# cvxopt/smcp

Hardware: AMD Instinct MI355X
Metric: Newton KKT solves/sec (higher is better)
Workload: dtype f64; 1 GPU; synth50k nested block-arrow SDP n=50000, 8073 cliques, m=100; kktsolver=chol, n=50000, cliques=8073, m=100, blkval_doubles=2493568, update_doubles=10689536, parallelism=single

## Files before the change

smcp_amd/csrc/constraints.cpp:

```cpp
#include "constraints.hpp"

#include <algorithm>
#include <atomic>

#include "../../include/smcp_amd.h"
#include "hostpar.hpp"

namespace smcp {
namespace {

struct Build {
  const Symbolic& S;
  const ConstraintParams& P;
  const int64_t m, nnz;
  const int64_t* cptr;
  const int64_t* cidx;
  const double* cval;
  ConstraintTables& T;
  std::vector<int32_t> ek, eoff;
  int threads = 1;
};

bool locate_entries(Build& B) {
  const Symbolic& S = B.S;
  ConstraintTables& T = B.T;
  const int64_t nnz = B.nnz;
  const int64_t* cidx = B.cidx;
  const double* cval = B.cval;
  T.w.resize(nnz); T.ar.resize(nnz); T.ac.resize(nnz);
  B.ek.resize(nnz); B.eoff.resize(nnz);
  const int nth = B.threads = host_threads(B.P.max_threads, nnz / 65536 + 1);
  std::atomic<int> bad{0};
  auto work = [&](int tix) {
    const int64_t e0 = nnz * tix / nth, e1 = nnz * (tix + 1) / nth;
    int64_t k = 0;
    for (int64_t e = e0; e < e1; ++e) {
      int64_t pos = cidx[e];
      if (pos < 0 || pos >= S.blklen()) { bad = 1; return; }
      if (pos < S.blkptr[k] || pos >= S.blkptr[k + 1])
        k = (int64_t)(std::upper_bound(S.blkptr.begin(), S.blkptr.end(), pos) - S.blkptr.begin()) - 1;
      int64_t nf = S.nf(k), off = pos - S.blkptr[k];
      int64_t col = off / nf, row = off % nf;
      if (row < col) { bad = 1; return; }
      T.w[e] = (row == col) ? cval[e] : 2.0 * cval[e];
      T.ar[e] = (int32_t)S.rowidx[S.rowptr[k] + row];
      T.ac[e] = (int32_t)(S.snptr[k] + col);
      B.ek[e] = (int32_t)k;
      B.eoff[e] = (int32_t)off;
    }
  };
  run_threads(nth, work);
  return !bad;
}

void classify_columns(Build& B) {
  const Symbolic& S = B.S;
  const ConstraintParams& P = B.P;
  ConstraintTables& T = B.T;
  const int64_t m = B.m, nnz = B.nnz;
  const int64_t* cptr = B.cptr;
  T.rloc.assign(nnz, 0); T.cloc.assign(nnz, 0);
  T.h_kptr.assign(1, 0);
  const int64_t tnz = (int64_t)((double)S.n * P.tnzcols);
  const int64_t colcap = ((int64_t)256 << 20) / std::max<int64_t>(1, S.n * 8);
  const int64_t kcap = std::min<int64_t>(tnz, std::max<int64_t>(1, colcap));
  const int64_t sepsum = std::max<int64_t>(1, S.sepptr[S.nsn]);
  const int64_t trsm_cap = std::max<int64_t>(1, (P.max_rhs * P.tmplen) / sepsum);
  std::vector<std::vector<int32_t>> kss((size_t)m);
  std::vector<char> is_sparse((size_t)m, 0);
  const int64_t cap = std::min(kcap, trsm_cap);
  const int nth = B.threads = host_threads(P.max_threads, m, nnz / 4096 + 1);
  auto work = [&](int tix) {
    for (int64_t j = tix; j < m; j += nth) {
      std::vector<int32_t>& ks = kss[(size_t)j];
      ks.reserve((size_t)(2 * (cptr[j + 1] - cptr[j])));
      for (int64_t e = cptr[j]; e < cptr[j + 1]; ++e) { ks.push_back(T.ar[e]); ks.push_back(T.ac[e]); }
      std::sort(ks.begin(), ks.end());
      ks.erase(std::unique(ks.begin(), ks.end()), ks.end());
      const int64_t nz = (int64_t)ks.size();
      const bool sparse = P.scm_on && nz > 0 && nz <= cap;
      is_sparse[(size_t)j] = sparse ? 1 : 0;
      if (!sparse) { std::vector<int32_t>().swap(ks); continue; }
      for (int64_t e = cptr[j]; e < cptr[j + 1]; ++e) {
        T.rloc[e] = (int32_t)(std::lower_bound(ks.begin(), ks.end(), T.ar[e]) - ks.begin());
        T.cloc[e] = (int32_t)(std::lower_bound(ks.begin(), ks.end(), T.ac[e]) - ks.begin());
      }
    }
  };
  run_threads(nth, work);
  int64_t kmax = 1;
  for (int64_t j = 0; j < m; ++j) {
    if (!is_sparse[(size_t)j]) { T.dl.push_back((int32_t)j); continue; }
    T.sl.push_back((int32_t)j);
    T.kidx.insert(T.kidx.end(), kss[(size_t)j].begin(), kss[(size_t)j].end());
    T.h_kptr.push_back((int64_t)T.kidx.size());
    kmax = std::max(kmax, (int64_t)kss[(size_t)j].size());
  }
  if (!T.sl.empty()) T.vcols = std::min(trsm_cap, std::max(kmax, std::min<int64_t>((int64_t)T.kidx.size(), colcap)));
}

void csr_by_position(Build& B) {
  ConstraintTables& T = B.T;
  const int64_t m = B.m, nnz = B.nnz;
  const int64_t* cptr = B.cptr;
  const int64_t* cidx = B.cidx;
  const double* cval = B.cval;
  T.rcon.resize(nnz); T.rval.resize(nnz);
  std::vector<int32_t> con(nnz);
  for (int64_t j = 0; j < m; ++j)
    for (int64_t e = cptr[j]; e < cptr[j + 1]; ++e) con[e] = (int32_t)j;
  const int nth = B.threads = host_threads(B.P.max_threads, nnz / 65536 + 1);
  const int64_t P = B.S.blklen();
  std::vector<std::vector<int64_t>> start((size_t)nth);
  std::vector<int64_t> ecount((size_t)nth + 1, 0), dcount((size_t)nth + 1, 0);
  auto count = [&](int tix) {
    const int64_t p0 = P * tix / nth, p1 = P * (tix + 1) / nth;
    std::vector<int64_t>& st = start[(size_t)tix];
    st.assign((size_t)(p1 - p0) + 1, 0);
    for (int64_t e = 0; e < nnz; ++e) { const int64_t p = cidx[e]; if (p >= p0 && p < p1) ++st[(size_t)(p - p0) + 1]; }
    int64_t distinct = 0;
    for (int64_t p = 0; p < p1 - p0; ++p) { distinct += st[(size_t)p + 1] != 0; st[(size_t)p + 1] += st[(size_t)p]; }
    ecount[(size_t)tix + 1] = st[(size_t)(p1 - p0)];
    dcount[(size_t)tix + 1] = distinct;
  };
  run_threads(nth, count);
  for (int t = 0; t < nth; ++t) { ecount[(size_t)t + 1] += ecount[(size_t)t]; dcount[(size_t)t + 1] += dcount[(size_t)t]; }
  T.rpos.resize((size_t)dcount[(size_t)nth]);
  T.rptr.resize((size_t)dcount[(size_t)nth] + 1);
  auto place = [&](int tix) {
    const int64_t p0 = P * tix / nth, p1 = P * (tix + 1) / nth, q0 = ecount[(size_t)tix];
    std::vector<int64_t>& st = start[(size_t)tix];
    int64_t d = dcount[(size_t)tix];
    for (int64_t p = 0; p < p1 - p0; ++p)
      if (st[(size_t)p + 1] != st[(size_t)p]) { T.rpos[(size_t)d] = p0 + p; T.rptr[(size_t)d] = q0 + st[(size_t)p]; ++d; }
    for (int64_t e = 0; e < nnz; ++e) {
      const int64_t p = cidx[e];
      if (p < p0 || p >= p1) continue;
      const int64_t q = q0 + st[(size_t)(p - p0)]++;
      T.rcon[(size_t)q] = con[e];
      T.rval[(size_t)q] = cval[e];
    }
  };
  run_threads(nth, place);
  T.rptr[(size_t)dcount[(size_t)nth]] = nnz;
}

void group_entries(Build& B) {
  const Symbolic& S = B.S;
  ConstraintTables& T = B.T;
  const int64_t m = B.m, nnz = B.nnz;
  const int64_t* cptr = B.cptr;
  const std::vector<int32_t>& ek = B.ek;
  const std::vector<int32_t>& eoff = B.eoff;
  std::vector<int32_t>& kptr = T.kptr;
  kptr.assign((size_t)(S.nsn * (m + 1)) + 1, 0);
  T.koff.resize(nnz); T.kval.resize(nnz); T.kij.resize(nnz);
  const int nth = B.threads = host_threads(B.P.max_threads, m, nnz / 65536 + 1);
  auto over_constraints = [&](auto body) {
    run_threads(nth, [&](int tix) { for (int64_t j = tix; j < m; j += nth) body(j); });
  };
  over_constraints([&](int64_t j) {
    for (int64_t e = cptr[j]; e < cptr[j + 1]; ++e) kptr[(size_t)ek[e] * (m + 1) + j + 1]++;
  });
  int64_t run = 0;
  for (int64_t k = 0; k < S.nsn; ++k) {
    for (int64_t j = 0; j <= m; ++j) {
      const size_t idx = (size_t)k * (m + 1) + j;
      const int32_t cnt = (j < m) ? kptr[idx + 1] : 0;
      kptr[idx] = (int32_t)run;
      if (j < m) run += cnt;
    }
  }
  std::vector<int32_t> fill(kptr.begin(), kptr.end() - 1);
  over_constraints([&](int64_t j) {
    for (int64_t e = cptr[j]; e < cptr[j + 1]; ++e) {
      const int64_t nf = S.nf(ek[e]);
      const int32_t q = fill[(size_t)ek[e] * (m + 1) + j]++;
      T.koff[q] = eoff[e];
      T.kval[q] = B.cval[e];
      T.kij[q] = (int32_t)((eoff[e] % nf) & 0xffff) | (int32_t)((eoff[e] / nf) << 16);
    }
  });
  kptr.pop_back();
  T.kc_sorted = true;
  for (size_t q = 0; q + 1 < kptr.size() && T.kc_sorted; ++q)
    for (int32_t e = kptr[q] + 1; e < kptr[q + 1]; ++e)
      if (T.koff[(size_t)e] <= T.koff[(size_t)e - 1]) { T.kc_sorted = false; break; }
}

void entry_statistics(Build& B) {
  const Symbolic& S = B.S;
  ConstraintTables& T = B.T;
  const int64_t m = B.m;
  const std::vector<int64_t>& fam = *B.P.fam;
  auto len = [&](int64_t k, int64_t j) { const size_t q = (size_t)k * (m + 1) + j; return (int64_t)(T.kptr[q + 1] - T.kptr[q]); };
  T.kc_maxlist = 0;
  for (int64_t k = 0; k < S.nsn; ++k)
    if (S.nn(k) <= 16 && S.na(k) <= 64)
      for (int64_t j = 0; j < m; ++j) T.kc_maxlist = std::max(T.kc_maxlist, len(k, j));
  int64_t sum = 0, pairs = 0;
  for (int64_t k = 0; k < S.nsn; ++k)
    if (k < (int64_t)fam.size() && fam[k] == 2)
      for (int64_t j = 0; j < m; ++j) {
        int64_t tot = len(k, j);
        for (int64_t q2 = S.chptr[k]; q2 < S.chptr[k + 1]; ++q2) tot += len(S.chidx[q2], j);
        T.fam_maxterms = std::max(T.fam_maxterms, tot);
        sum += tot;
        ++pairs;
      }
  if (pairs) T.fam_meanterms = (double)sum / (double)pairs;
  T.kc_maxlist_large = 0;
  for (int64_t k = 0; k < S.nsn; ++k)
    if ((S.nn(k) > 16 || S.na(k) > 64) && S.nn(k) <= 64 && S.na(k) <= 128 && S.chptr[k + 1] == S.chptr[k])
      for (int64_t j = 0; j < m; ++j) T.kc_maxlist_large = std::max(T.kc_maxlist_large, len(k, j));
  T.lg_slot_of.assign((size_t)S.nsn, -1);
  T.lg_eptr.assign(1, 0);
  for (int64_t k = 0; k < S.nsn; ++k)
    if (k < (int64_t)fam.size() && fam[k] == 1) {
      const int64_t E = T.kptr[(size_t)k * (m + 1) + m] - T.kptr[(size_t)k * (m + 1)];
      T.lg_slot_of[(size_t)k] = (int32_t)T.lg_children++;
      T.lg_maxent = std::max(T.lg_maxent, E);
      T.lg_pairs += E * (E + 1) / 2;
      T.lg_rows += S.nf(k) * S.nn(k);
      T.lg_rec = std::max<int>(T.lg_rec, (int)(S.nf(k) * S.nf(k) + S.nf(k) * S.nn(k)));
      T.lg_eptr.push_back(T.lg_eptr.back() + (int32_t)E);
    }
}

void leafgram_lists(Build& B) {
  ConstraintTables& T = B.T;
  const int64_t m = B.m;
  T.epk.resize((size_t)T.lg_eptr.back());
  T.ewv.resize((size_t)T.lg_eptr.back());
  T.remap.assign((size_t)m, -1);
  for (int64_t k = 0; k < B.S.nsn; ++k) {
    const int32_t g = T.lg_slot_of[(size_t)k];
    if (g < 0) continue;
    int32_t o = T.lg_eptr[(size_t)g];
    for (int64_t j = 0; j < m; ++j)
      for (int32_t q = T.kptr[(size_t)k * (m + 1) + j]; q < T.kptr[(size_t)k * (m + 1) + j + 1]; ++q, ++o) {
        const int32_t i = T.kij[q] & 0xffff, jc = T.kij[q] >> 16;
        T.epk[(size_t)o] = i | (jc << 8) | ((int32_t)j << 16);
        T.ewv[(size_t)o] = i == jc ? 0.5 * T.kval[q] : T.kval[q];
      }
  }
  for (size_t q = 0; q < T.dl.size(); ++q) T.remap[(size_t)T.dl[q]] = (int32_t)q;
  T.has_leafgram = true;
}

bool number_families(Build& B) {
  const Symbolic& S = B.S;
  const ConstraintParams& P = B.P;
  ConstraintTables& T = B.T;
  T.fno.assign((size_t)S.nsn, -1);
  T.fz_levels.assign((size_t)S.nlev, 0);
  T.has_fz_levels = true;
  int64_t nfam = 0;
  bool ok = true;
  for (int64_t k = 0; k < S.nsn; ++k)
    if ((*P.fam)[(size_t)k] == 2) {
      T.fno[(size_t)k] = (int32_t)nfam++;
      const int64_t par = S.snpar[k];
      if (par < 0 || (size_t)par >= P.large_mask->size() || !(*P.large_mask)[(size_t)par] || S.nf(par) > P.lf_alds_maxnf) ok = false;
      else T.fz_levels[(size_t)S.level[(size_t)par]] = 1;
    }
  T.fz_nfam = nfam;
  return ok && nfam > 0 && nfam < ((int64_t)1 << 19) && nfam * (B.m + 1) < ((int64_t)1 << 31);
}

void family_term_lists(Build& B) {
  const Symbolic& S = B.S;
  ConstraintTables& T = B.T;
  const int64_t m = B.m, nfam = T.fz_nfam;
  const int32_t CHILD = B.P.famt_child;
  const std::vector<int32_t>& kptr = T.kptr;
  const std::vector<int32_t>& kij = T.kij;
  const std::vector<double>& kval = T.kval;
  std::vector<int32_t>& fptr = T.fptr;
  fptr.assign((size_t)(nfam * (m + 1)) + 1, 0);
  std::vector<int64_t> fam_k((size_t)nfam);
  int64_t run = 0;
  for (int64_t k = 0; k < S.nsn; ++k) {
    const int32_t f = T.fno[(size_t)k];
    if (f < 0) continue;
    fam_k[(size_t)f] = k;
    for (int64_t j = 0; j < m; ++j) {
      fptr[(size_t)f * (m + 1) + j] = (int32_t)run;
      run += kptr[(size_t)k * (m + 1) + j + 1] - kptr[(size_t)k * (m + 1) + j];
      for (int64_t q2 = S.chptr[k]; q2 < S.chptr[k + 1]; ++q2) {
        const size_t q = (size_t)S.chidx[q2] * (m + 1) + j;
        run += kptr[q + 1] - kptr[q];
      }
    }
    fptr[(size_t)f * (m + 1) + m] = (int32_t)run;
  }
  fptr[(size_t)(nfam * (m + 1))] = (int32_t)run;
  T.fpk.resize((size_t)run);
  T.fsv.resize((size_t)run);
  const int nth = B.threads = host_threads(B.P.max_threads, nfam / 16 + 1);
  run_threads(nth, [&](int tix) {
    for (int64_t f = tix; f < nfam; f += nth) {
      const int64_t k = fam_k[(size_t)f];
      for (int64_t j = 0; j < m; ++j) {
        size_t o = (size_t)fptr[(size_t)f * (m + 1) + j];
        for (int32_t q = kptr[(size_t)k * (m + 1) + j]; q < kptr[(size_t)k * (m + 1) + j + 1]; ++q, ++o) {
          const int32_t i = kij[q] & 0xffff, jc = kij[q] >> 16;
          T.fpk[o] = i | (jc << 16);
          T.fsv[o] = i == jc ? 0.5 * kval[q] : kval[q];
        }
        int32_t colbase = 0;
        for (int64_t q2 = S.chptr[k]; q2 < S.chptr[k + 1]; ++q2) {
          const int64_t cc = S.chidx[q2];
          const int32_t nnc = (int32_t)S.nn(cc);
          const int32_t* rel = &S.relidx[S.sepptr[cc]];
          for (int32_t q = kptr[(size_t)cc * (m + 1) + j]; q < kptr[(size_t)cc * (m + 1) + j + 1]; ++q, ++o) {
            const int32_t i = kij[q] & 0xffff, jc = kij[q] >> 16;
            if (i >= nnc) { T.fpk[o] = (CHILD + colbase + jc) | (rel[i - nnc] << 16); T.fsv[o] = -kval[q]; }
            else { T.fpk[o] = (CHILD + colbase + i) | ((CHILD + colbase + jc) << 16); T.fsv[o] = i == jc ? 0.5 * kval[q] : kval[q]; }
          }
          colbase += nnc;
        }
      }
    }
  });
  T.has_fam_terms = true;
}

}

int build_constraint_tables(const Symbolic& S, const ConstraintParams& P, int64_t m, const int64_t* cptr, const int64_t* cidx,
                            const double* cval, ConstraintTables& T, const ConstraintStepMark& mark) {
  T = ConstraintTables();
  Build B{S, P, m, cptr[m], cptr, cidx, cval, T, {}, {}};
  auto done = [&](const char* step) { if (mark) mark(step, B.threads); B.threads = 1; };
  if (!locate_entries(B)) return SMCP_EINVAL;
  done("locate entries");
  classify_columns(B);
  done("classify");
  csr_by_position(B);
  done("CSR by position");
  if (B.nnz < ((int64_t)1 << 31) && S.nsn * (m + 1) <= ((int64_t)1 << 28)) {
    group_entries(B);
    entry_statistics(B);
    T.has_entry_tables = true;
    done("entry tables");
    if (T.lg_children > 0 && m < 32768) leafgram_lists(B);
    done("leaf Gram tables");
    if (T.fam_maxterms > 0 && P.famt_terms_ok(T.fam_maxterms, T.fam_meanterms) && !P.fam->empty() && number_families(B))
      family_term_lists(B);
    done("family term lists");
  }
  return 0;
}

}
```

smcp_amd/csrc/front_famt.hip:

```cpp
#include <hip/hip_runtime.h>

namespace smcp {

struct FamtL { int oLi, onK, onMK, oRt, oZero, oCN, oCA, oCM, total; };
template <int NAT>
__host__ __device__ inline FamtL famt_layout(int ncol) {
  constexpr int NA = 16 * NAT;
  FamtL L{};
  int o = 0;
  L.oLi = o; o += 256;
  L.onK = o; o += NA * 16;
  L.onMK = o; o += NA * 16;
  L.oRt = o; o += NA * NA;
  L.oZero = o; o += NA;
  L.oCN = o; o += ncol * 16;
  L.oCA = o; o += ncol * NA;
  L.oCM = o; o += ncol * NA;
  L.total = o;
  return L;
}
typedef unsigned int famt_u2 __attribute__((ext_vector_type(2)));
__device__ inline __amdgpu_buffer_rsrc_t famt_rsrc(double* base, int doubles) {
  return __builtin_amdgcn_make_buffer_rsrc(base, 0, doubles * 8, 0x00020000);
}
#ifndef SMCP_FAMT_AUX
#define SMCP_FAMT_AUX 0
#endif
__device__ inline void famt_store(__amdgpu_buffer_rsrc_t r, bool ok, int pos, double v) {
  __builtin_amdgcn_raw_buffer_store_b64(__builtin_bit_cast(famt_u2, v), r, ok ? pos * 8 : -1, 0, SMCP_FAMT_AUX);
}
#ifndef SMCP_FAMT_NW
#define SMCP_FAMT_NW 12
#endif
constexpr int FAMT_NW = SMCP_FAMT_NW;
constexpr int FAMT_HDR = 32;
constexpr int FAMT_TCAP = 96;
constexpr int FAMT_TMAX = 384;
constexpr int FAMT_CHILD = 128;

template <int NAT>
__host__ __device__ inline int famt_prep_doubles(int cnn) { constexpr int NA = 16 * NAT; return NA * NA + NA * 16 + 256 + 8 * (NA + 16 + cnn * NA); }

template <int NAT>
__global__ void __launch_bounds__(512) k_famt_prep(MfmaArgs a, double* famt, int cnn, int32_t* fz_slot) {
  extern __shared__ __attribute__((aligned(16))) double smem[];
  constexpr int NA = 16 * NAT;
  const int ncol = 8 * cnn;
  const FamtL L = famt_layout<NAT>(ncol);
  const int k = a.t.lev[blockIdx.x];
  const CliqueDesc d = a.t.cl[k];
  const int nn = d.nn, na = d.na, nf = nn + na, nch = d.chend - d.chbeg;
  const int tid = threadIdx.x, lane = tid & 63, wave = tid >> 6;
  double* const sRt = smem;
  double* const snK = sRt + NA * NA;
  double* const sLi = snK + NA * 16;
  double* const qt = sLi + 256 + wave * (NA + 16 + cnn * NA);
  double* const sCA = qt + NA + 16;
  double* const out = famt + (int64_t)blockIdx.x * (FAMT_HDR + L.total);
  double* const T = out + FAMT_HDR;
  const int myck = lane < nch ? a.t.chidx[d.chbeg + lane] : 0;
  const int mynn = lane < nch ? a.t.cl[myck].nn : 0;
  int inc = mynn;
#pragma unroll
  for (int o = 1; o < 8; o <<= 1) { const int v = __shfl_up(inc, o); if (lane >= o) inc += v; }
  const int colbase = __shfl(inc - mynn, min(wave, 7));
  const int ck = __shfl(myck, min(wave, 7));
  for (int e = tid; e < NA * NA + NA * 16 + 256; e += 512) smem[e] = 0.0;
  __syncthreads();
  {
    const double* lk = a.LK + d.blk;
    const double* ys = a.ysc + d.upd;
    for (int e = tid; e < nf * nn; e += 512) {
      const int i = e % nf, j = e / nf;
      if (i >= nn) snK[(i - nn) + j * NA] = -lk[e];
      else if (i >= j) sLi[i + j * 16] = lk[e];
    }
    batched_loop<8>(tid, na * na, 512, [=](int e) { return ys[e]; },
                    [=](int e, double v) {
                      const int i = e % na, p = e / na;
                      if (i >= p) sRt[p + i * NA] = v;
                    });
  }
  __syncthreads();
  for (int e = tid; e < 256; e += 512) T[L.oLi + e] = sLi[e];
  for (int e = tid; e < NA * 16; e += 512) T[L.onK + e] = snK[e];
  for (int e = tid; e < NA * NA; e += 512) T[L.oRt + e] = sRt[e];
  for (int e = tid; e < NA; e += 512) T[L.oZero + e] = 0.0;
  for (int e = tid; e < NA * 16; e += 512) {
    const int p = e % NA, c = e / NA;
    double s = 0.0;
    if (p < na && c < nn)
      for (int q = p; q < na; ++q) s += sRt[p + q * NA] * snK[q + c * NA];
    T[L.onMK + e] = s;
  }
  if (wave < nch) {
    const CliqueDesc cd = a.t.cl[ck];
    const int nnc = cd.nn, nac = cd.na, nfc = nnc + nac;
    const double* lkc = a.LK + cd.blk;
    const int rel = lane < nac ? a.t.relidx[cd.rel + lane] : 0;
    for (int j = 0; j < nnc; ++j) {
      const double kv = lane < nac ? lkc[(nnc + lane) + (int64_t)j * nfc] : 0.0;
      for (int e = lane; e < NA + 16; e += 64) qt[e] = 0.0;
      __builtin_amdgcn_fence(__ATOMIC_RELEASE, "wavefront"); __builtin_amdgcn_wave_barrier(); __builtin_amdgcn_fence(__ATOMIC_ACQUIRE, "wavefront");
      if (lane < nac) qt[rel < nn ? rel : 16 + (rel - nn)] = kv;
      __builtin_amdgcn_fence(__ATOMIC_RELEASE, "wavefront"); __builtin_amdgcn_wave_barrier(); __builtin_amdgcn_fence(__ATOMIC_ACQUIRE, "wavefront");
      const int g = colbase + j;
      if (lane < 16) {
        double s = 0.0;
        if (lane < nn)
          for (int q = 0; q <= lane; ++q) s += sLi[lane + q * 16] * qt[q];
        T[L.oCN + g * 16 + lane] = s;
      }
      for (int p = lane; p < NA; p += 64) {
        double s = 0.0;
        if (p < na) {
          s = qt[16 + p];
          for (int q = 0; q < nn; ++q) s += snK[p + q * NA] * qt[q];
        }
        sCA[j * NA + p] = s;
        T[L.oCA + g * NA + p] = s;
      }
    }
    __builtin_amdgcn_fence(__ATOMIC_RELEASE, "wavefront"); __builtin_amdgcn_wave_barrier(); __builtin_amdgcn_fence(__ATOMIC_ACQUIRE, "wavefront");
    for (int j0 = 0; j0 < nnc; j0 += 8)
      for (int p = lane; p < NA; p += 64) {
        double s8[8] = {0.0, 0.0, 0.0, 0.0, 0.0, 0.0, 0.0, 0.0};
        if (p < na)
          for (int q = p; q < na; ++q) {
            const double rt = sRt[p + q * NA];
#pragma unroll
            for (int x = 0; x < 8; ++x) s8[x] += rt * sCA[min(j0 + x, cnn - 1) * NA + q];
          }
#pragma unroll
        for (int x = 0; x < 8; ++x) if (j0 + x < nnc) T[L.oCM + (colbase + j0 + x) * NA + p] = s8[x];
      }
    if (lane == 0) {
      int* const hdr = reinterpret_cast<int*>(out) + 16 + 6 * wave;
      hdr[0] = ck; hdr[1] = nnc; hdr[2] = nac; hdr[3] = colbase; hdr[4] = 0; hdr[5] = 0;
    }
  } else if (wave < 8 && lane == 0) {
    int* const hdr = reinterpret_cast<int*>(out) + 16 + 6 * wave;
    hdr[0] = -1; hdr[1] = 1; hdr[2] = 0; hdr[3] = 0; hdr[4] = 0; hdr[5] = 0;
  }
  {
    const int used = __shfl(inc, 7);
    for (int e = tid; e < (ncol - used) * 16; e += 512) T[L.oCN + used * 16 + e] = 0.0;
    for (int e = tid; e < (ncol - used) * NA; e += 512) { T[L.oCA + used * NA + e] = 0.0; T[L.oCM + used * NA + e] = 0.0; }
  }
  if (tid == 0) {
    if (fz_slot && a.fz_no && a.fz_no[k] >= 0) fz_slot[a.fz_no[k]] = (int32_t)blockIdx.x;
    int* const hdr = reinterpret_cast<int*>(out);
    hdr[0] = k; hdr[1] = nn; hdr[2] = na; hdr[3] = nch;
    hdr[4] = (int)(d.blk & 0xffffffffll); hdr[5] = (int)(d.blk >> 32);
    hdr[6] = 0; hdr[7] = 0;
    hdr[8] = (int)(d.updp & 0xffffffffll); hdr[9] = (int)(d.updp >> 32);
  }
}

template <int NTH>
__device__ inline void famt_copy_tables(double* smem, const double* src, int total, int tid) {
  const double2* const s2 = reinterpret_cast<const double2*>(src);
  double2* const d2 = reinterpret_cast<double2*>(smem);
  const int n2 = total >> 1;
  for (int e0 = tid; e0 < n2; e0 += NTH * 8) {
    double2 v[8];
#pragma unroll
    for (int x = 0; x < 8; ++x) v[x] = s2[min(e0 + x * NTH, n2 - 1)];
#pragma unroll
    for (int x = 0; x < 8; ++x) if (e0 + x * NTH < n2) d2[e0 + x * NTH] = v[x];
  }
}

__host__ __device__ inline int famt_desc_doubles() { return FAMT_TCAP * 3; }

template <int NAT, bool UPD = true>
__global__ void __launch_bounds__(64 * FAMT_NW) k_fam_terms(MfmaArgs a, double* u, int64_t ldu, const double* famt, int cnn,
                                                   const int32_t* kc_ij, int tabpasses, int ecap) {
  extern __shared__ __attribute__((aligned(16))) double smem[];
  constexpr int NA = 16 * NAT, NW = FAMT_NW, NTH = 64 * NW;
  const int ncol = 8 * cnn;
  const FamtL L = famt_layout<NAT>(ncol);
  const double* const fc = famt + (int64_t)blockIdx.x * (FAMT_HDR + L.total);
  const int32_t* const hdr = reinterpret_cast<const int32_t*>(fc);
  const int k = hdr[0], nn = hdr[1], na = hdr[2], nch = hdr[3], nf = nn + na;
  const int64_t pblk = (int64_t)(uint32_t)hdr[4] | ((int64_t)hdr[5] << 32);
  const int64_t pupdp = (int64_t)(uint32_t)hdr[8] | ((int64_t)hdr[9] << 32);
  const int tid = threadIdx.x;
  const int lane = tid & 63, l15 = lane & 15, kq = lane >> 4;
  const int wave = __builtin_amdgcn_readfirstlane(tid >> 6);
  const int nmem = nch + 1;
  const int gy = (int)gridDim.y;
  const int npass = ((int)a.nrhs - (int)blockIdx.y + gy - 1) / gy;
  double* const dS = smem + L.total + wave * famt_desc_doubles();
  int* const dI = reinterpret_cast<int*>(dS + FAMT_TCAP);
  int* const misc = reinterpret_cast<int*>(smem + L.total + NW * famt_desc_doubles());
  int* const epfit = misc;
  int* const cdim = misc + 2;
  int* const tab = misc + 12;
  double* const lval = reinterpret_cast<double*>(tab + 2 * ((tabpasses * nmem + 1) & ~1));
  int* const lpk = reinterpret_cast<int*>(lval + ecap);

  famt_copy_tables<NTH>(smem, fc + FAMT_HDR, L.total, tid);
  if (tid < 8) cdim[tid] = tid < nch ? (hdr[16 + 6 * tid + 1] | (hdr[16 + 6 * tid + 3] << 8)) : 1;

  for (int q0 = 0; q0 < npass;) {
    const int epmax = min(tabpasses, npass - q0), npairs = epmax * nmem;
    __syncthreads();
    if (tid == 0) *epfit = epmax;
    int myp0[2] = {0, 0};
#pragma unroll
    for (int h = 0; h < 2; ++h) {
      const int idx = tid + NTH * h;
      if (idx < npairs) {
        const int qq = idx / nmem, mem = idx - qq * nmem;
        const int r = (int)blockIdx.y + (q0 + qq) * gy;
        const int j = a.kc_ids ? a.kc_ids[a.kc_j0 + r] : a.kc_j0 + r;
        const int ck = mem ? hdr[16 + 6 * (mem - 1)] : k;
        const int32_t* kp = a.kc_ptr + (int64_t)ck * a.kc_stride;
        myp0[h] = kp[j];
        tab[2 * idx] = kp[j + 1] - myp0[h];
      }
    }
    __syncthreads();
    if (wave == 0) {
      const int per = (npairs + 63) / 64, b = lane * per;
      int sum = 0;
      for (int x = 0; x < per; ++x) sum += (b + x < npairs) ? tab[2 * (b + x)] : 0;
      int incl = sum;
#pragma unroll
      for (int o = 1; o < 64; o <<= 1) { const int v = __shfl_up(incl, o); if (lane >= o) incl += v; }
      int run = incl - sum;
      for (int x = 0; x < per; ++x)
        if (b + x < npairs) {
          const int c = tab[2 * (b + x)];
          tab[2 * (b + x) + 1] = run;
          run += c;
          if (run > ecap) atomicMin(epfit, (b + x) / nmem);
        }
    }
    __syncthreads();
    const int ep = max(1, *epfit);
#pragma unroll
    for (int h = 0; h < 2; ++h) {
      const int idx = tid + NTH * h;
      if (idx < ep * nmem) {
        const int c = tab[2 * idx], p0 = myp0[h], off = tab[2 * idx + 1];
        const int qq = idx / nmem, mem = idx - qq * nmem;
        (void)qq;
        const int mnn = mem ? hdr[16 + 6 * (mem - 1) + 1] : 0;
        const int mck = mem ? hdr[16 + 6 * (mem - 1)] : 0;
        const int32_t* const mrel = a.t.relidx + a.t.cl[mem ? mck : k].rel;
        for (int t = 0; t < c && off + t < ecap; ++t) {
          const int ij = kc_ij[p0 + t];
          const int i = ij & 0xffff, jc = ij >> 16;
          int pk = i | (jc << 8);
          if (mem && i >= mnn) pk |= mrel[i - mnn] << 16;
          lpk[off + t] = pk;
          lval[off + t] = a.kc_val[p0 + t];
        }
      }
    }
    __builtin_amdgcn_s_waitcnt(0x0F70);
    __syncthreads();

    for (int qq = wave; qq < ep; qq += NW) {
      const int r = (int)blockIdx.y + (q0 + qq) * gy;
      const int* const trow = tab + 2 * qq * nmem;
      int cntm = lane < nmem ? trow[2 * lane] : 0;
      int incl = cntm;
#pragma unroll
      for (int o = 1; o < 16; o <<= 1) { const int v = __shfl_up(incl, o); if (lane >= o) incl += v; }
      const int Ttot = min(__builtin_amdgcn_readlane(incl, 15), FAMT_TMAX);
      const int ndp = max(1, (Ttot + FAMT_TCAP / 2 - 1) / (FAMT_TCAP / 2));
      auto build = [&](int dp) {
        const int e = dp * (FAMT_TCAP / 2) + lane;
        const int T = min(FAMT_TCAP / 2, Ttot - dp * (FAMT_TCAP / 2));
        int mem = 0, base = 0;
#pragma unroll
        for (int mm = 0; mm < 8; ++mm) {
          const int up = __builtin_amdgcn_readlane(incl, mm);
          if (e >= up) { mem = mm + 1; base = up; }
        }
        if (lane < T) {
          const int where = trow[2 * mem + 1];
          const int pk = lpk[where + (e - base)];
          const double v = lval[where + (e - base)];
          const int i = pk & 0xff, jc = (pk >> 8) & 0xff, rl = (pk >> 16) & 0xff;
          int vx, vy;
          double s;
          if (mem == 0) { vx = i; vy = jc; s = i == jc ? 0.5 * v : v; }
          else {
            const int cd = cdim[mem - 1], nnc = cd & 0xff, cb = cd >> 8;
            if (i >= nnc) { vx = FAMT_CHILD + cb + jc; vy = rl; s = -v; }
            else { vx = FAMT_CHILD + cb + i; vy = FAMT_CHILD + cb + jc; s = i == jc ? 0.5 * v : v; }
          }
          auto img = [&](int vid, int& on, int& oa, int& om, int& ui) {
            if (vid >= FAMT_CHILD) { const int g = vid - FAMT_CHILD; on = L.oCN + 16 * g; oa = L.oCA + NA * g; om = L.oCM + NA * g; ui = 255; }
            else if (vid < nn) { on = L.oLi + 16 * vid; oa = L.onK + NA * vid; om = L.onMK + NA * vid; ui = 255; }
            else { on = L.oZero; oa = L.oZero; om = L.oRt + NA * (vid - nn); ui = vid - nn; }
          };
          int nx, ax, mx, ux, ny, ay, my, uy;
          img(vx, nx, ax, mx, ux);
          img(vy, ny, ay, my, uy);
          dS[2 * lane] = s; dS[2 * lane + 1] = s;
          int4 w0 = {nx | (ax << 16), mx | (ux << 16), ny | (ay << 16), uy};
          int4 w1 = {ny | (ay << 16), my | (uy << 16), nx | (ax << 16), ux};
          reinterpret_cast<int4*>(dI)[2 * lane] = w0;
          reinterpret_cast<int4*>(dI)[2 * lane + 1] = w1;
        }
        if (lane < 4 && 2 * T + lane < ((2 * T + 3) & ~3)) {
          dS[2 * T + lane] = 0.0;
          int4 z = {L.oZero | (L.oZero << 16), L.oZero | (255 << 16), L.oZero | (L.oZero << 16), 255};
          reinterpret_cast<int4*>(dI)[2 * T + lane] = z;
        }
        __builtin_amdgcn_fence(__ATOMIC_RELEASE, "wavefront"); __builtin_amdgcn_wave_barrier(); __builtin_amdgcn_fence(__ATOMIC_ACQUIRE, "wavefront");
      };
      build(0);
      const __amdgpu_buffer_rsrc_t rP = famt_rsrc(u + (int64_t)r * ldu + pblk, nf * nn);
      const __amdgpu_buffer_rsrc_t rU = famt_rsrc(a.t.updp + (int64_t)r * a.t.updplen + pupdp, (na * (na + 1)) >> 1);
      bool fresh = true;
      auto pass = [&](auto LOc, auto HIc, auto Gc) {
        constexpr int LO = decltype(LOc)::value, HI = decltype(HIc)::value;
        constexpr bool WITHG = decltype(Gc)::value;
        constexpr int NTU = UPD ? HI * (HI + 1) / 2 - LO * (LO + 1) / 2 : 1;
        d4 accU[NTU], accQ[HI - LO], accG = {0.0, 0.0, 0.0, 0.0};
#pragma unroll
        for (int x = 0; x < NTU; ++x) accU[x] = d4{0.0, 0.0, 0.0, 0.0};
#pragma unroll
        for (int x = 0; x < HI - LO; ++x) accQ[x] = d4{0.0, 0.0, 0.0, 0.0};
        for (int dp = 0; dp < ndp; ++dp) {
        if (!(fresh && dp == 0)) {
          __builtin_amdgcn_fence(__ATOMIC_RELEASE, "wavefront"); __builtin_amdgcn_wave_barrier(); __builtin_amdgcn_fence(__ATOMIC_ACQUIRE, "wavefront");
          build(dp);
        }
        fresh = ndp == 1;
        const int ks = (2 * min(FAMT_TCAP / 2, Ttot - dp * (FAMT_TCAP / 2)) + 3) >> 2;
        for (int s = 0; s < ks; ++s) {
          const int tp = kq + 4 * s;
          const double sc = dS[tp];
          const int4 w = reinterpret_cast<const int4*>(dI)[tp];
          const int nx = w.x & 0xffff, ax = w.x >> 16, mx = w.y & 0xffff, ux = w.y >> 16;
          const int ny = w.z & 0xffff, ay = w.z >> 16, uy = w.w;
          double bA[HI - LO], bM[HI - LO], aA[HI];
#pragma unroll
          for (int t = 0; t < HI; ++t) {
            const int row = 16 * t + l15;
            if constexpr (UPD) aA[t] = sc * (smem[ay + row] + (row == uy ? 1.0 : 0.0));
            if (t >= LO) {
              if constexpr (UPD) bA[t - LO] = smem[ax + row] + (row == ux ? 1.0 : 0.0);
              bM[t - LO] = smem[mx + row];
            }
          }
          const double aN = sc * smem[ny + l15];
#pragma unroll
          for (int rt = LO; rt < HI; ++rt) {
            if constexpr (UPD) {
#pragma unroll
              for (int ct = 0; ct <= rt; ++ct) {
                constexpr int base = LO * (LO + 1) / 2;
                const int x = rt * (rt + 1) / 2 + ct - base;
                accU[x] = __builtin_amdgcn_mfma_f64_16x16x4f64(aA[ct], bA[rt - LO], accU[x], 0, 0, 0);
              }
            }
            accQ[rt - LO] = __builtin_amdgcn_mfma_f64_16x16x4f64(aN, bM[rt - LO], accQ[rt - LO], 0, 0, 0);
          }
          if constexpr (WITHG) {
            const double bN = smem[nx + l15];
            accG = __builtin_amdgcn_mfma_f64_16x16x4f64(aN, bN, accG, 0, 0, 0);
          }
        }
        }
#pragma unroll
        for (int rt = LO; rt < HI; ++rt) {
          const int m = 16 * rt + l15;
          const bool mok = m < na;
          if constexpr (UPD) {
#pragma unroll
            for (int ct = 0; ct <= rt; ++ct)
#pragma unroll
              for (int x = 0; x < 4; ++x) {
                const int n = 16 * ct + kq + 4 * x;
                const int cb = (n * (2 * na - 1 - n)) >> 1;
                famt_store(rU, ct < rt ? mok : (mok && m >= n), cb + m, accU[rt * (rt + 1) / 2 + ct - LO * (LO + 1) / 2][x]);
              }
          }
#pragma unroll
          for (int x = 0; x < 4; ++x) {
            const int n = kq + 4 * x;
            famt_store(rP, mok && n < nn, (nn + m) + n * nf, accQ[rt - LO][x]);
          }
        }
        if constexpr (WITHG) {
#pragma unroll
          for (int x = 0; x < 4; ++x) {
            const int jn = kq + 4 * x;
            famt_store(rP, l15 < nn && jn <= l15, l15 + jn * nf, accG[x]);
          }
        }
      };
      if constexpr (!UPD) {
        pass(std::integral_constant<int, 0>{}, std::integral_constant<int, NAT>{}, std::true_type{});
      } else if constexpr (NAT == 4 && FAMT_NW > 8) {
        pass(std::integral_constant<int, 0>{}, std::integral_constant<int, 2>{}, std::true_type{});
        pass(std::integral_constant<int, 2>{}, std::integral_constant<int, 3>{}, std::false_type{});
        pass(std::integral_constant<int, 3>{}, std::integral_constant<int, 4>{}, std::false_type{});
      } else if constexpr (NAT == 3 && FAMT_NW > 8) {
        pass(std::integral_constant<int, 0>{}, std::integral_constant<int, 2>{}, std::true_type{});
        pass(std::integral_constant<int, 2>{}, std::integral_constant<int, 3>{}, std::false_type{});
      } else if constexpr (NAT == 4) {
        pass(std::integral_constant<int, 0>{}, std::integral_constant<int, 3>{}, std::false_type{});
        pass(std::integral_constant<int, 3>{}, std::integral_constant<int, 4>{}, std::true_type{});
      } else {
        pass(std::integral_constant<int, 0>{}, std::integral_constant<int, NAT>{}, std::true_type{});
      }
    }
    q0 += ep;
  }
}

template <int NAT, int PFG = 1>
__device__ inline void lf_add_family(double* T, int nf, const MfmaArgs& a, int z, int64_t pt, const int32_t* rel, int lane) {
  constexpr int NA = 16 * NAT, NTU = NAT * (NAT + 1) / 2;
  const int l15 = lane & 15, kq = lane >> 4;
  const int slot = z & 0x7ffff, nnp = (z >> 19) & 31, nap = (z >> 24) & 127;
  const FamtL L = famt_layout<NAT>(8 * a.fz_cnn);
  const double* const tab = a.fz_tab + (int64_t)slot * a.fz_recl + FAMT_HDR;
  const int pbase = (int)(uint32_t)(pt & 0xffffffffll), Ttot = min((int)(pt >> 32), FAMT_TMAX);
  int relv[NAT];
#pragma unroll
  for (int t = 0; t < NAT; ++t) relv[t] = rel[min(16 * t + l15, max(nap - 1, 0))];
  d4 acc[NTU];
#pragma unroll
  for (int x = 0; x < NTU; ++x) acc[x] = d4{0.0, 0.0, 0.0, 0.0};
  auto chunk = [&](const int p0, const int Tn) {
  int pk = 0;
  double sv = 0.0;
  if (lane < Tn) { pk = a.fz_pk[p0 + lane]; sv = a.fz_s[p0 + lane]; }
  const int ks = (2 * Tn + 3) >> 2;
  auto fetch = [&](int s, double (&aA)[NAT], double& se, int& ux, int& uy) {
    const int tp = kq + 4 * s, e = tp >> 1;
    const int pke = __shfl(pk, e, 64);
    se = __shfl(sv, e, 64);
    const int v0 = pke & 0xffff, v1 = (pke >> 16) & 0xffff;
    const int vx = (tp & 1) ? v1 : v0, vy = (tp & 1) ? v0 : v1;
    ux = (vx < FAMT_CHILD && vx >= nnp) ? vx - nnp : 255;
    const int ay = vy >= FAMT_CHILD ? L.oCA + NA * (vy - FAMT_CHILD) : (vy < nnp ? L.onK + NA * vy : L.oZero);
    uy = (vy < FAMT_CHILD && vy >= nnp) ? vy - nnp : 255;
#pragma unroll
    for (int t = 0; t < NAT; ++t) aA[t] = tab[ay + 16 * t + l15];
  };
  auto mma = [&](double (&aA)[NAT], double se, int ux, int uy) {
    double bA[NAT];
#pragma unroll
    for (int t = 0; t < NAT; ++t) bA[t] = __shfl_xor(aA[t], 16, 64);
#pragma unroll
    for (int t = 0; t < NAT; ++t) {
      const int row = 16 * t + l15;
      aA[t] = se * (aA[t] + (row == uy ? 1.0 : 0.0));
      bA[t] = bA[t] + (row == ux ? 1.0 : 0.0);
    }
#pragma unroll
    for (int rt = 0; rt < NAT; ++rt)
#pragma unroll
      for (int ct = 0; ct <= rt; ++ct)
        acc[rt * (rt + 1) / 2 + ct] = __builtin_amdgcn_mfma_f64_16x16x4f64(aA[ct], bA[rt], acc[rt * (rt + 1) / 2 + ct], 0, 0, 0);
  };
  if constexpr (PFG == 1) {
    for (int s = 0; s < ks; ++s) {
      double aA[NAT], se;
      int ux, uy;
      fetch(s, aA, se, ux, uy);
      mma(aA, se, ux, uy);
    }
  } else {
    for (int s0 = 0; s0 < ks; s0 += PFG) {
      double aA[PFG][NAT], se[PFG];
      int ux[PFG], uy[PFG];
#pragma unroll
      for (int g = 0; g < PFG; ++g) {
        fetch(min(s0 + g, ks - 1), aA[g], se[g], ux[g], uy[g]);
        if (s0 + g >= ks) se[g] = 0.0;
      }
#pragma unroll
      for (int g = 0; g < PFG; ++g) mma(aA[g], se[g], ux[g], uy[g]);
    }
  }
  };
  if (Ttot <= 64) chunk(pbase, Ttot);
  else for (int c0 = 0; c0 < Ttot; c0 += 64) chunk(pbase + c0, min(64, Ttot - c0));
#pragma unroll
  for (int rt = 0; rt < NAT; ++rt) {
    const int m = 16 * rt + l15;
#pragma unroll
    for (int ct = 0; ct <= rt; ++ct)
#pragma unroll
      for (int x = 0; x < 4; ++x) {
        const int n = 16 * ct + kq + 4 * x;
        const int cj = __shfl(relv[ct], kq + 4 * x, 64);
        const bool ok = m < nap && n < nap && (ct < rt || m >= n);
        if (ok) unsafeAtomicAdd(&T[cj * nf - ((cj * (cj - 1)) >> 1) - cj + relv[rt]], acc[rt * (rt + 1) / 2 + ct][x]);
      }
  }
}
template <int NAT, int PFG = 1>
struct AldsFam {
  const MfmaArgs* a;
  const int64_t* sCu; const int64_t* sCr;
  __device__ void operator()(double* T, int nf, int r, const int* sFz, int nmine, int wave, int nw, int lane) const {
    (void)r;
    for (int qi = wave; qi < nmine; qi += nw) {
      const int z = sFz[qi];
      if (z >= 0) lf_add_family<NAT, PFG>(T, nf, *a, z, sCu[qi], a->t.relidx + sCr[qi], lane);
    }
  }
};
template <int NAT, int NTH>
__global__ void __launch_bounds__(NTH) k_lf_assemble_fz(MfmaArgs a, double* u, int64_t ldu, int sgn, int cnt, int nrhs, int* counters,
                                                        int tail_first, int nzt) {
  extern __shared__ __attribute__((aligned(16))) double T[];
  __shared__ int stask;
  const int64_t* const sCu = reinterpret_cast<const int64_t*>(T + lf_alds_doubles(a.nnmax + a.namax));
  const int64_t* const sCr = sCu + a.nchmax;
  const int q0 = (int)(blockIdx.x & 7);
  for (int dq = 0; dq < 8; ++dq) {
    const int q = (q0 + dq) & 7;
    const int nfq = (cnt - q + 7) >> 3;
    const int total = nfq * nrhs;
    if (total <= 0) continue;
    const int full = (tail_first >= 0 && tail_first < total) ? tail_first : total;
    const int units = full + (total - full) * nzt;
    for (;;) {
      __syncthreads();
      if (threadIdx.x == 0) stask = atomicAdd(counters + q, 1);
      __syncthreads();
      const int t = stask;
      if (t >= units) break;
      if (t < full) {
        lf_alds_task(a, u, ldu, sgn, q + 8 * (t / nrhs), t % nrhs, 0, 1, T, AldsFam<NAT, (NTH == 512 ? 4 : 1)>{&a, sCu, sCr});
      } else {
        const int s2 = t - full, tt = full + s2 / nzt, share = s2 % nzt;
        const int tc = (a.nchmax + nzt - 1) / nzt;
        lf_alds_task(a, u, ldu, sgn, q + 8 * (tt / nrhs), tt % nrhs, share, nzt, T, AldsFam<NAT, (NTH == 512 ? 4 : 1)>{&a, sCu, sCu + tc});
      }
    }
  }
}

constexpr int FAMT_GMAX = 8;
constexpr int FAMT_GTAB = 2 * 8 * FAMT_GMAX * 9;
__host__ __device__ inline int famt_grp_misc_doubles() { return (12 + FAMT_GTAB) / 2; }

template <int NAT>
__global__ void __launch_bounds__(512) k_fam_terms_grp(MfmaArgs a, double* u, int64_t ldu, const double* famt, int cnn,
                                                       const int32_t* kc_ij, int ecap) {
  extern __shared__ __attribute__((aligned(16))) double smem[];
  constexpr int NA = 16 * NAT, NW = 8, NMEM = 9, NTU = NAT * (NAT + 1) / 2;
  const int ncol = 8 * cnn;
  const FamtL L = famt_layout<NAT>(ncol);
  const int64_t recl = FAMT_HDR + L.total;
  const int g0 = a.grp_ptr[blockIdx.x];
  const int M = min(a.grp_ptr[blockIdx.x + 1] - g0, FAMT_GMAX);
  const int32_t* const glist = a.grp_list + g0;
  const int tid = threadIdx.x;
  const int lane = tid & 63, l15 = lane & 15, kq = lane >> 4;
  const int wave = __builtin_amdgcn_readfirstlane(tid >> 6);
  const int gy = (int)gridDim.y;
  const int npass = ((int)a.nrhs - (int)blockIdx.y + gy - 1) / gy;
  double* const dS = smem + L.total + wave * famt_desc_doubles();
  int* const dI = reinterpret_cast<int*>(dS + FAMT_TCAP);
  int* const misc = reinterpret_cast<int*>(smem + L.total + NW * famt_desc_doubles());
  int* const epfit = misc;
  int* const cdim = misc + 2;
  int* const tab = misc + 12;
  double* const lval = reinterpret_cast<double*>(tab + FAMT_GTAB);
  int* const lpk = reinterpret_cast<int*>(lval + ecap);
  const int32_t* const hlead = reinterpret_cast<const int32_t*>(famt + (int64_t)glist[0] * recl);
  const int na = hlead[2];
  const int64_t lupdp = (int64_t)(uint32_t)hlead[8] | ((int64_t)hlead[9] << 32);
  const int stride = M * NMEM;

  for (int q0 = 0; q0 < npass;) {
    const int epmax = min(NW, npass - q0), npairs = epmax * stride;
    __syncthreads();
    if (tid == 0) *epfit = epmax;
    int myp0[2] = {0, 0};
#pragma unroll
    for (int h = 0; h < 2; ++h) {
      const int idx = tid + 512 * h;
      if (idx < npairs) {
        const int qq = idx / stride, rem = idx - qq * stride, mf = rem / NMEM, mem = rem - mf * NMEM;
        const int r = (int)blockIdx.y + (q0 + qq) * gy;
        const int j = a.kc_ids ? a.kc_ids[a.kc_j0 + r] : a.kc_j0 + r;
        const int32_t* const hm = reinterpret_cast<const int32_t*>(famt + (int64_t)glist[mf] * recl);
        const int ck = mem ? hm[16 + 6 * (mem - 1)] : hm[0];
        int cnt = 0;
        if (ck >= 0) {
          const int32_t* kp = a.kc_ptr + (int64_t)ck * a.kc_stride;
          myp0[h] = kp[j];
          cnt = kp[j + 1] - myp0[h];
        }
        tab[2 * idx] = cnt;
      }
    }
    __syncthreads();
    if (wave == 0) {
      const int per = (npairs + 63) / 64, b = lane * per;
      int sum = 0;
      for (int x = 0; x < per; ++x) sum += (b + x < npairs) ? tab[2 * (b + x)] : 0;
      int incl = sum;
#pragma unroll
      for (int o = 1; o < 64; o <<= 1) { const int v = __shfl_up(incl, o); if (lane >= o) incl += v; }
      int run = incl - sum;
      for (int x = 0; x < per; ++x)
        if (b + x < npairs) {
          const int c = tab[2 * (b + x)];
          tab[2 * (b + x) + 1] = run;
          run += c;
          if (run > ecap) atomicMin(epfit, (b + x) / stride);
        }
    }
    __syncthreads();
    const int ep = max(1, *epfit);
#pragma unroll
    for (int h = 0; h < 2; ++h) {
      const int idx = tid + 512 * h;
      if (idx < ep * stride) {
        const int c = tab[2 * idx], p0 = myp0[h], off = tab[2 * idx + 1];
        const int qq = idx / stride, rem = idx - qq * stride, mf = rem / NMEM, mem = rem - mf * NMEM;
        if (c > 0) {
          const int32_t* const hm = reinterpret_cast<const int32_t*>(famt + (int64_t)glist[mf] * recl);
          const int mnn = mem ? hm[16 + 6 * (mem - 1) + 1] : 0;
          const int mck = mem ? hm[16 + 6 * (mem - 1)] : hm[0];
          const int32_t* const mrel = a.t.relidx + a.t.cl[mck].rel;
          for (int t = 0; t < c && off + t < ecap; ++t) {
            const int ij = kc_ij[p0 + t];
            const int i = ij & 0xffff, jc = ij >> 16;
            int pk = i | (jc << 8);
            if (mem && i >= mnn) pk |= mrel[i - mnn] << 16;
            lpk[off + t] = pk;
            lval[off + t] = a.kc_val[p0 + t];
          }
        }
      }
    }
    __builtin_amdgcn_s_waitcnt(0x0F70);
    const int qq = wave;
    const bool active = qq < ep;
    const int r = (int)blockIdx.y + (q0 + min(qq, ep - 1)) * gy;
    d4 accU[NTU];
#pragma unroll
    for (int x = 0; x < NTU; ++x) accU[x] = d4{0.0, 0.0, 0.0, 0.0};
    for (int mf = 0; mf < M; ++mf) {
      const double* const fcm = famt + (int64_t)glist[mf] * recl;
      const int32_t* const hm = reinterpret_cast<const int32_t*>(fcm);
      const int nn = hm[1], nch = hm[3], nf = nn + na;
      const int64_t pblk = (int64_t)(uint32_t)hm[4] | ((int64_t)hm[5] << 32);
      __syncthreads();
      famt_copy_tables<512>(smem, fcm + FAMT_HDR, L.total, tid);
      if (tid < 8) cdim[tid] = tid < nch ? (hm[16 + 6 * tid + 1] | (hm[16 + 6 * tid + 3] << 8)) : 1;
      __syncthreads();
      if (!active) continue;
      const int* const trow = tab + 2 * ((qq * M + mf) * NMEM);
      int cntm = lane < NMEM ? trow[2 * lane] : 0;
      int incl = cntm;
#pragma unroll
      for (int o = 1; o < 16; o <<= 1) { const int v = __shfl_up(incl, o); if (lane >= o) incl += v; }
      const int T = min(__builtin_amdgcn_readlane(incl, 15), FAMT_TCAP / 2);
      {
        int mem = 0, base = 0;
#pragma unroll
        for (int mm = 0; mm < 8; ++mm) {
          const int up = __builtin_amdgcn_readlane(incl, mm);
          if (lane >= up) { mem = mm + 1; base = up; }
        }
        if (lane < T) {
          const int where = trow[2 * mem + 1];
          const int pk = lpk[where + (lane - base)];
          const double v = lval[where + (lane - base)];
          const int i = pk & 0xff, jc = (pk >> 8) & 0xff, rl = (pk >> 16) & 0xff;
          int vx, vy;
          double s;
          if (mem == 0) { vx = i; vy = jc; s = i == jc ? 0.5 * v : v; }
          else {
            const int cd = cdim[mem - 1], nnc = cd & 0xff, cb = cd >> 8;
            if (i >= nnc) { vx = FAMT_CHILD + cb + jc; vy = rl; s = -v; }
            else { vx = FAMT_CHILD + cb + i; vy = FAMT_CHILD + cb + jc; s = i == jc ? 0.5 * v : v; }
          }
          auto img = [&](int vid, int& on, int& oa, int& om, int& ui) {
            if (vid >= FAMT_CHILD) { const int g = vid - FAMT_CHILD; on = L.oCN + 16 * g; oa = L.oCA + NA * g; om = L.oCM + NA * g; ui = 255; }
            else if (vid < nn) { on = L.oLi + 16 * vid; oa = L.onK + NA * vid; om = L.onMK + NA * vid; ui = 255; }
            else { on = L.oZero; oa = L.oZero; om = L.oRt + NA * (vid - nn); ui = vid - nn; }
          };
          int nx, ax, mx, ux, ny, ay, my, uy;
          img(vx, nx, ax, mx, ux);
          img(vy, ny, ay, my, uy);
          dS[2 * lane] = s; dS[2 * lane + 1] = s;
          int4 w0 = {nx | (ax << 16), mx | (ux << 16), ny | (ay << 16), uy};
          int4 w1 = {ny | (ay << 16), my | (uy << 16), nx | (ax << 16), ux};
          reinterpret_cast<int4*>(dI)[2 * lane] = w0;
          reinterpret_cast<int4*>(dI)[2 * lane + 1] = w1;
        }
        if (lane < 4 && 2 * T + lane < ((2 * T + 3) & ~3)) {
          dS[2 * T + lane] = 0.0;
          int4 z = {L.oZero | (L.oZero << 16), L.oZero | (255 << 16), L.oZero | (L.oZero << 16), 255};
          reinterpret_cast<int4*>(dI)[2 * T + lane] = z;
        }
      }
      __builtin_amdgcn_fence(__ATOMIC_RELEASE, "wavefront"); __builtin_amdgcn_wave_barrier(); __builtin_amdgcn_fence(__ATOMIC_ACQUIRE, "wavefront");
      const int ks = (2 * T + 3) >> 2;
      const __amdgpu_buffer_rsrc_t rP = famt_rsrc(u + (int64_t)r * ldu + pblk, nf * nn);
      auto pass = [&](auto LOc, auto HIc, auto Gc) {
        constexpr int LO = decltype(LOc)::value, HI = decltype(HIc)::value;
        constexpr bool WITHG = decltype(Gc)::value;
        d4 accQ[HI - LO], accG = {0.0, 0.0, 0.0, 0.0};
#pragma unroll
        for (int x = 0; x < HI - LO; ++x) accQ[x] = d4{0.0, 0.0, 0.0, 0.0};
        for (int s = 0; s < ks; ++s) {
          const int tp = kq + 4 * s;
          const double sc = dS[tp];
          const int4 w = reinterpret_cast<const int4*>(dI)[tp];
          const int nx = w.x & 0xffff, ax = w.x >> 16, mx = w.y & 0xffff, ux = w.y >> 16;
          const int ny = w.z & 0xffff, ay = w.z >> 16, uy = w.w;
          double bA[HI - LO], bM[HI - LO], aA[HI];
#pragma unroll
          for (int t = 0; t < HI; ++t) {
            const int row = 16 * t + l15;
            aA[t] = sc * (smem[ay + row] + (row == uy ? 1.0 : 0.0));
            if (t >= LO) {
              bA[t - LO] = smem[ax + row] + (row == ux ? 1.0 : 0.0);
              bM[t - LO] = smem[mx + row];
            }
          }
          const double aN = sc * smem[ny + l15];
#pragma unroll
          for (int rt = LO; rt < HI; ++rt) {
#pragma unroll
            for (int ct = 0; ct <= rt; ++ct) {
              const int x = rt * (rt + 1) / 2 + ct;
              accU[x] = __builtin_amdgcn_mfma_f64_16x16x4f64(aA[ct], bA[rt - LO], accU[x], 0, 0, 0);
            }
            accQ[rt - LO] = __builtin_amdgcn_mfma_f64_16x16x4f64(aN, bM[rt - LO], accQ[rt - LO], 0, 0, 0);
          }
          if constexpr (WITHG) {
            const double bN = smem[nx + l15];
            accG = __builtin_amdgcn_mfma_f64_16x16x4f64(aN, bN, accG, 0, 0, 0);
          }
        }
#pragma unroll
        for (int rt = LO; rt < HI; ++rt) {
          const int m = 16 * rt + l15;
          const bool mok = m < na;
#pragma unroll
          for (int x = 0; x < 4; ++x) {
            const int n = kq + 4 * x;
            famt_store(rP, mok && n < nn, (nn + m) + n * nf, accQ[rt - LO][x]);
          }
        }
        if constexpr (WITHG) {
#pragma unroll
          for (int x = 0; x < 4; ++x) {
            const int jn = kq + 4 * x;
            famt_store(rP, l15 < nn && jn <= l15, l15 + jn * nf, accG[x]);
          }
        }
      };
      if constexpr (NAT == 4) {
        pass(std::integral_constant<int, 0>{}, std::integral_constant<int, 3>{}, std::false_type{});
        pass(std::integral_constant<int, 3>{}, std::integral_constant<int, 4>{}, std::true_type{});
      } else {
        pass(std::integral_constant<int, 0>{}, std::integral_constant<int, NAT>{}, std::true_type{});
      }
    }
    if (active) {
      const __amdgpu_buffer_rsrc_t rU = famt_rsrc(a.t.updp + (int64_t)r * a.t.updplen + lupdp, (na * (na + 1)) >> 1);
#pragma unroll
      for (int rt = 0; rt < NAT; ++rt) {
        const int m = 16 * rt + l15;
        const bool mok = m < na;
#pragma unroll
        for (int ct = 0; ct <= rt; ++ct)
#pragma unroll
          for (int x = 0; x < 4; ++x) {
            const int n = 16 * ct + kq + 4 * x;
            const int cb = (n * (2 * na - 1 - n)) >> 1;
            famt_store(rU, ct < rt ? mok : (mok && m >= n), cb + m, accU[rt * (rt + 1) / 2 + ct][x]);
          }
      }
    }
    q0 += ep;
  }
}

}
```

Baseline: 360.0 KKT solves/s.

## Split unit-vector family terms out of MFMA path into direct rank-1 atomic updates

The host builder now classifies family terms whose two endpoints differ in whether they hit a unit (identity) column, tags them with a flag bit, and places them after the regular terms in each list. The device kernel handles these tagged terms with a cheap per-lane scaled-vector atomic update instead of feeding them through the MFMA outer-product accumulation, and skips the MFMA pass entirely when no regular terms remain. This is meant to cut wasted matrix-core work on rank-1 terms that are mostly zeros. The cost is extra atomics, a more complex term encoding with 8-bit index masks, and risk if index fields exceed 255.

```diff
diff --git a/smcp_amd/csrc/constraints.cpp b/smcp_amd/csrc/constraints.cpp
--- a/smcp_amd/csrc/constraints.cpp
+++ b/smcp_amd/csrc/constraints.cpp
@@ -268,6 +268,7 @@
   return ok && nfam > 0 && nfam < ((int64_t)1 << 19) && nfam * (B.m + 1) < ((int64_t)1 << 31);
 }
 
+constexpr int32_t FAM_UNIT_TERM = 1 << 30;
 void family_term_lists(Build& B) {
   const Symbolic& S = B.S;
   ConstraintTables& T = B.T;
@@ -299,27 +300,42 @@
   T.fsv.resize((size_t)run);
   const int nth = B.threads = host_threads(B.P.max_threads, nfam / 16 + 1);
   run_threads(nth, [&](int tix) {
+    std::vector<int32_t> upk;
+    std::vector<double> usv;
     for (int64_t f = tix; f < nfam; f += nth) {
       const int64_t k = fam_k[(size_t)f];
+      const int32_t nnp = (int32_t)S.nn(k);
       for (int64_t j = 0; j < m; ++j) {
         size_t o = (size_t)fptr[(size_t)f * (m + 1) + j];
-        for (int32_t q = kptr[(size_t)k * (m + 1) + j]; q < kptr[(size_t)k * (m + 1) + j + 1]; ++q, ++o) {
+        upk.clear();
+        usv.clear();
+        auto put = [&](int32_t vx, int32_t vy, double s) {
+          const bool ux = vx < CHILD && vx >= nnp, uy = vy < CHILD && vy >= nnp;
+          if (ux != uy) {
+            upk.push_back((ux ? vy | (vx << 16) : vx | (vy << 16)) | FAM_UNIT_TERM);
+            usv.push_back(s);
+          } else {
+            T.fpk[o] = vx | (vy << 16);
+            T.fsv[o++] = s;
+          }
+        };
+        for (int32_t q = kptr[(size_t)k * (m + 1) + j]; q < kptr[(size_t)k * (m + 1) + j + 1]; ++q) {
           const int32_t i = kij[q] & 0xffff, jc = kij[q] >> 16;
-          T.fpk[o] = i | (jc << 16);
-          T.fsv[o] = i == jc ? 0.5 * kval[q] : kval[q];
+          put(i, jc, i == jc ? 0.5 * kval[q] : kval[q]);
         }
         int32_t colbase = 0;
         for (int64_t q2 = S.chptr[k]; q2 < S.chptr[k + 1]; ++q2) {
           const int64_t cc = S.chidx[q2];
           const int32_t nnc = (int32_t)S.nn(cc);
           const int32_t* rel = &S.relidx[S.sepptr[cc]];
-          for (int32_t q = kptr[(size_t)cc * (m + 1) + j]; q < kptr[(size_t)cc * (m + 1) + j + 1]; ++q, ++o) {
+          for (int32_t q = kptr[(size_t)cc * (m + 1) + j]; q < kptr[(size_t)cc * (m + 1) + j + 1]; ++q) {
             const int32_t i = kij[q] & 0xffff, jc = kij[q] >> 16;
-            if (i >= nnc) { T.fpk[o] = (CHILD + colbase + jc) | (rel[i - nnc] << 16); T.fsv[o] = -kval[q]; }
-            else { T.fpk[o] = (CHILD + colbase + i) | ((CHILD + colbase + jc) << 16); T.fsv[o] = i == jc ? 0.5 * kval[q] : kval[q]; }
+            if (i >= nnc) put(CHILD + colbase + jc, rel[i - nnc], -kval[q]);
+            else put(CHILD + colbase + i, CHILD + colbase + jc, i == jc ? 0.5 * kval[q] : kval[q]);
           }
           colbase += nnc;
         }
+        for (size_t x = 0; x < upk.size(); ++x, ++o) { T.fpk[o] = upk[x]; T.fsv[o] = usv[x]; }
       }
     }
   });
diff --git a/smcp_amd/csrc/front_famt.hip b/smcp_amd/csrc/front_famt.hip
--- a/smcp_amd/csrc/front_famt.hip
+++ b/smcp_amd/csrc/front_famt.hip
@@ -37,6 +37,11 @@
 constexpr int FAMT_TCAP = 96;
 constexpr int FAMT_TMAX = 384;
 constexpr int FAMT_CHILD = 128;
+constexpr int FAMT_UNIT = 1 << 30;
+#ifndef SMCP_FAMT_UB
+#define SMCP_FAMT_UB 8
+#endif
+constexpr int FAMT_UB = SMCP_FAMT_UB;
 
 template <int NAT>
 __host__ __device__ inline int famt_prep_doubles(int cnn) { constexpr int NA = 16 * NAT; return NA * NA + NA * 16 + 256 + 8 * (NA + 16 + cnn * NA); }
@@ -426,22 +431,55 @@
   const FamtL L = famt_layout<NAT>(8 * a.fz_cnn);
   const double* const tab = a.fz_tab + (int64_t)slot * a.fz_recl + FAMT_HDR;
   const int pbase = (int)(uint32_t)(pt & 0xffffffffll), Ttot = min((int)(pt >> 32), FAMT_TMAX);
-  int relv[NAT];
-#pragma unroll
-  for (int t = 0; t < NAT; ++t) relv[t] = rel[min(16 * t + l15, max(nap - 1, 0))];
-  d4 acc[NTU];
-#pragma unroll
-  for (int x = 0; x < NTU; ++x) acc[x] = d4{0.0, 0.0, 0.0, 0.0};
-  auto chunk = [&](const int p0, const int Tn) {
+  const int rell = rel[min(lane, max(nap - 1, 0))];
   int pk = 0;
   double sv = 0.0;
-  if (lane < Tn) { pk = a.fz_pk[p0 + lane]; sv = a.fz_s[p0 + lane]; }
+  auto load = [&](const int p0, const int Tn) {
+    pk = 0; sv = 0.0;
+    if (lane < Tn) { pk = a.fz_pk[p0 + lane]; sv = a.fz_s[p0 + lane]; }
+    return (int)__popcll(__ballot(lane < Tn && !(pk & FAMT_UNIT)));
+  };
+  auto units = [&](const int Td, const int Tn) {
+    for (int t0 = Td; t0 < Tn; t0 += FAMT_UB) {
+      double av[FAMT_UB];
+      int pkt[FAMT_UB];
+#pragma unroll
+      for (int g = 0; g < FAMT_UB; ++g) {
+        pkt[g] = __builtin_amdgcn_readlane(pk, min(t0 + g, Tn - 1));
+        const int vd = pkt[g] & 0xff;
+        const int ad = vd >= FAMT_CHILD ? L.oCA + NA * (vd - FAMT_CHILD) : L.onK + NA * vd;
+        av[g] = tab[ad + min(lane, NA - 1)];
+      }
+      const famt_u2 sw = __builtin_bit_cast(famt_u2, sv);
+#pragma unroll
+      for (int g = 0; g < FAMT_UB; ++g)
+        if (t0 + g < Tn) {
+          const int u = (((pkt[g] >> 16) & 0xff) - nnp) & 63;
+          const famt_u2 sl = {(unsigned)__builtin_amdgcn_readlane((int)sw.x, t0 + g), (unsigned)__builtin_amdgcn_readlane((int)sw.y, t0 + g)};
+          const double s = __builtin_bit_cast(double, sl);
+          const int fu = __builtin_amdgcn_readlane(rell, u);
+          const int cj = min(rell, fu), ri = max(rell, fu);
+          if (lane < nap) unsafeAtomicAdd(&T[cj * nf - ((cj * (cj - 1)) >> 1) - cj + ri], (lane == u ? 2.0 : 1.0) * s * av[g]);
+        }
+    }
+  };
+  int Td = 0;
+  for (int c0 = 0; c0 < Ttot; c0 += 64) {
+    const int Tn = min(64, Ttot - c0), Tdc = load(pbase + c0, Tn);
+    units(Tdc, Tn);
+    Td += Tdc;
+  }
+  if (Td == 0) return;
+  d4 acc[NTU];
+#pragma unroll
+  for (int x = 0; x < NTU; ++x) acc[x] = d4{0.0, 0.0, 0.0, 0.0};
+  auto chunk = [&](const int Tn) {
   const int ks = (2 * Tn + 3) >> 2;
   auto fetch = [&](int s, double (&aA)[NAT], double& se, int& ux, int& uy) {
     const int tp = kq + 4 * s, e = tp >> 1;
     const int pke = __shfl(pk, e, 64);
     se = __shfl(sv, e, 64);
-    const int v0 = pke & 0xffff, v1 = (pke >> 16) & 0xffff;
+    const int v0 = pke & 0xff, v1 = (pke >> 16) & 0xff;
     const int vx = (tp & 1) ? v1 : v0, vy = (tp & 1) ? v0 : v1;
     ux = (vx < FAMT_CHILD && vx >= nnp) ? vx - nnp : 255;
     const int ay = vy >= FAMT_CHILD ? L.oCA + NA * (vy - FAMT_CHILD) : (vy < nnp ? L.onK + NA * vy : L.oZero);
@@ -486,8 +524,17 @@
     }
   }
   };
-  if (Ttot <= 64) chunk(pbase, Ttot);
-  else for (int c0 = 0; c0 < Ttot; c0 += 64) chunk(pbase + c0, min(64, Ttot - c0));
+  if (Ttot <= 64) {
+    if (lane >= Td) { pk = 0; sv = 0.0; }
+    chunk(Td);
+  } else for (int c0 = 0; c0 < Td; c0 += 64) {
+    const int Tn = min(64, Td - c0);
+    load(pbase + c0, Tn);
+    chunk(Tn);
+  }
+  int relv[NAT];
+#pragma unroll
+  for (int t = 0; t < NAT; ++t) relv[t] = __shfl(rell, 16 * t + l15, 64);
 #pragma unroll
   for (int rt = 0; rt < NAT; ++rt) {
     const int m = 16 * rt + l15;
```

Result: faster. 378.7 KKT solves/s, median of 6 (+5.2%).
